# HamidGadirov/OpticalFlowSciVis

Hardware: AMD Instinct MI355X
Metric: volume-pairs/sec, Flow-3D unsupervised train step (fwd+loss+bwd+AdamW) (higher is better)
Workload: dtype f32

## Files before the change

opticalflowscivis_amd/csrc/convtr.hip:

```cpp
#include <cstdint>
#include <cstdlib>

#include "common.hpp"

namespace {

typedef float f32x16 __attribute__((ext_vector_type(16)));

struct TP {
  int B, Cin, Cout;
  int CoutT;
  int Di, Hi, Wi;
  int Dout, Hout, Wout;
  int Dq, Hq, Wq;
  int tz, ty, tx;
  long long tiles;
  const float* slope;
  float* Z;
  int nslope;
  const float* addend;
  const float* Ybase;
  long long wslice;
#ifdef FS_ABLATION
  int ab = 0;
// ... 589 lines not shown
  const int qz = qz0 + wz, qy = qy0 + wy;
  if (qz < p.Dq && qy < p.Hq) {
    const size_t yvol = (size_t)p.Dout * p.Hout * p.Wout;
#pragma unroll
    for (int n = 0; n < 2; ++n) {
      const int qx = qx0 + 16 * n + col;
#pragma unroll
      for (int r = 0; r < 4; ++r) {
        const int co = 4 * kq + r;
        const bool ok = co < p.Cout;
        const int cc = ok ? co : 0;
        const float bv = (bias && ok) ? bias[cc] : 0.f;
        float v[8];
#pragma unroll
        for (int c = 0; c < 8; ++c) v[c] = acc[n][c][r] + bv;
        store8_quad(Y + ((size_t)b * p.Cout + cc) * yvol, v, qz, qy, qx, ok, p,
                    p.Z ? p.Z + ((size_t)b * p.Cout + cc) * yvol : nullptr, p.Z ? p.slope[p.nslope == 1 ? 0 : cc] : 0.f);
      }
    }
  }
}

constexpr int p8_ws_ci(int rt) { return 128 * rt + 16; }
__host__ __device__ constexpr int p8_k(int par, int d) { return par == 0 ? (d == 0 ? 1 : 3) : (d == 0 ? 0 : 2); }

#ifdef FS_TR_STAMPS
__device__ unsigned long long fs_tr_dbg[4 * 8];
#define TSTAMP(i) do { const unsigned long long now_ = __builtin_amdgcn_s_memtime(); dt[i] += now_ - tprev; tprev = now_; } while (0)
#else
#define TSTAMP(i) do { } while (0)
#endif

template <int RT, int NT, int CINP>
__global__ __launch_bounds__(512, 2) void convtr_p8_kernel(const float* __restrict__ X, const float* __restrict__ Wt,
                                                        const float* __restrict__ bias, float* __restrict__ Y,
                                                        TP p, int per) {
  constexpr int CI = 4, XB = 16 * (NT - 1);
  constexpr int ZT = 3, YT = 3, XP = XB + 16;
  constexpr int PS = YT * XP;
  constexpr int CHS = ZT * PS + ((ZT * PS) % 32 == 16 ? 0 : 16);
  constexpr int NX = CI * CHS;
  constexpr int NXL = (NX + 255) / 256 * 256;
  constexpr int WSCI = p8_ws_ci(RT);
  constexpr int NW = CINP * WSCI;
  constexpr int NWL = (NW + 255) / 256 * 256;
  static_assert((NWL + 2 * NXL) * 4 <= 160 * 1024, "weights + two input buffers fit the CU's LDS");
  static_assert(NT % 2 == 1, "tiles are processed in pairs + one");
  __shared__ __attribute__((aligned(16))) float lds[NWL + 2 * NXL];

  const int t = threadIdx.x, lane = t & 63;
  const int wave = __builtin_amdgcn_readfirstlane(t >> 6);
  const int wv = wave & 3;
  const long long t0 = (long long)blockIdx.x * per, t1 = min(t0 + per, p.tiles);
  const size_t xvol = (size_t)p.Di * p.Hi * p.Wi;
  auto decode = [&](long long tile, int& b, int& qz0, int& qy0, int& q0) {
    const int txi = (int)(tile % p.tx); tile /= p.tx;
    const int tyi = (int)(tile % p.ty); tile /= p.ty;
    const int tzi = (int)(tile % p.tz);
    b = (int)(tile / p.tz);
    qz0 = tzi * 2; qy0 = tyi * 2; q0 = txi * XB;
  };

  if (wave >= 4) {
#if defined(__HIP_DEVICE_COMPILE__)
    __builtin_amdgcn_s_setprio(3);
    constexpr int NXW = (NXL / 256 + 3) / 4, NWW = (NWL / 256 + 3) / 4;
    {
      __amdgpu_buffer_rsrc_t rw = __builtin_amdgcn_make_buffer_rsrc((void*)Wt, (short)0, (p.Cin + 3) / 4 * 4 * WSCI * 4,
                                                                     0x00020000);
#pragma unroll
      for (int k = 0; k < NWW; ++k)
        if (256 * (wv + 4 * k) < NWL)
          __builtin_amdgcn_raw_ptr_buffer_load_lds(rw, (lds_ptr_t)(lds + 256 * (wv + 4 * k)), 16,
                                                   (unsigned)(256 * (wv + 4 * k) + 4 * lane) * 4u, 0, 0, 0);
    }
    unsigned xoff[NXW];
    int b = 0;
    auto offsets = [&](long long tile) {
      int qz0, qy0, q0;
      decode(tile, b, qz0, qy0, q0);
#pragma unroll
      for (int k = 0; k < NXW; ++k) {
        const int i = 256 * (wv + 4 * k) + 4 * lane;
        const int c = i / CHS, r1 = i - c * CHS;
        const int z = r1 / PS, r2 = r1 - z * PS;
        const int y = r2 / XP, x = r2 - y * XP;
        const int gz = qz0 - 1 + z, gy = qy0 - 1 + y, gx = q0 - 4 + x;
        const bool ok = i < NX && z < ZT && gz >= 0 && gz < p.Di && gy >= 0 && gy < p.Hi && gx >= 0 && gx < p.Wi;
// ... 38 lines not shown

  const int col = lane & 15, kq = lane >> 4;
  const int wz = wv >> 1, wy = wv & 1;
  const int bBo = NWL + kq * CHS + (wz + 1) * PS + (wy + 1) * XP + (col + 4);
  __builtin_amdgcn_s_barrier();
  int buf = 0;
#ifdef FS_TR_STAMPS
  unsigned long long dt[8] = {0, 0, 0, 0, 0, 0, 0, 0};
  unsigned long long tprev = __builtin_amdgcn_s_memtime();
#endif
  for (long long tile = t0; tile < t1; ++tile) {
    int b, qz0, qy0, q0;
    decode(tile, b, qz0, qy0, q0);
    const int qend = (q0 + XB >= p.Wi) ? p.Wi + 1 : q0 + XB;
    f32x4 acc[RT][NT];
#pragma unroll
    for (int rt = 0; rt < RT; ++rt)
#pragma unroll
      for (int n = 0; n < NT; ++n)
#pragma unroll
        for (int r = 0; r < 4; ++r) acc[rt][n][r] = 0.f;

    for (int c0 = 0; c0 < p.Cin; c0 += CI) {
      const float* aB = lds + (size_t)(c0 + kq) * WSCI + col;
      float av[8][RT];
#pragma unroll
      for (int d = 0; d < 8; ++d)
#pragma unroll
        for (int rt = 0; rt < RT; ++rt) av[d][rt] = aB[(d * RT + rt) * 16];
      const float* bB = lds + bBo + buf * NXL;
      float xa[2][8], xb[2][8];
      auto load_x = [&](int n, float (&xn)[8]) {
#pragma unroll
        for (int d = 0; d < 8; ++d) xn[d] = bB[16 * n - ((d >> 2) & 1) * PS - ((d >> 1) & 1) * XP - (d & 1)];
      };
      auto mma_pair = [&](int n, const float (&x0)[8], const float (&x1)[8], bool two) {
#pragma unroll
        for (int d = 0; d < 8; ++d)
#pragma unroll
          for (int rt = 0; rt < RT; ++rt) {
            acc[rt][n] = __builtin_amdgcn_mfma_f32_16x16x4f32(av[d][rt], x0[d], acc[rt][n], 0, 0, 0);
            if (two) acc[rt][n + 1] = __builtin_amdgcn_mfma_f32_16x16x4f32(av[d][rt], x1[d], acc[rt][n + 1], 0, 0, 0);
          }
      };
      load_x(0, xa[0]);
      if (NT > 1) load_x(1, xa[1]);
#pragma unroll
      for (int n = 0; n < NT; n += 4) {
        if (n + 2 < NT) { load_x(n + 2, xb[0]); if (n + 3 < NT) load_x(n + 3, xb[1]); }
        __builtin_amdgcn_sched_barrier(0);
        mma_pair(n, xa[0], xa[1], n + 1 < NT);
        if (n + 2 < NT) {
          if (n + 4 < NT) { load_x(n + 4, xa[0]); if (n + 5 < NT) load_x(n + 5, xa[1]); }
          __builtin_amdgcn_sched_barrier(0);
          mma_pair(n + 2, xb[0], xb[1], n + 3 < NT);
        }
      }
      TSTAMP(0);
      __builtin_amdgcn_s_barrier();
      TSTAMP(1);
      buf ^= 1;
    }

    const int qz = qz0 + wz, qy = qy0 + wy;
    if (qz <= p.Di && qy <= p.Hi) {
      const size_t yvol = (size_t)p.Dout * p.Hout * p.Wout;
      const bool evn = (col & 1) == 0;
      const int slot = 4 * (kq & 1) + (evn ? 0 : 1) + 2 * (lane >> 5);
#pragma unroll
      for (int rt = 0; rt < RT; ++rt) {
        const int item = 8 * rt + slot;
        const int pzy = item / p.Cout, co = item - pzy * p.Cout;
        const int zo = 2 * qz - (pzy >> 1), yo = 2 * qy - (pzy & 1);
        const bool iok = item < 4 * p.Cout && zo >= 0 && zo < p.Dout && yo >= 0 && yo < p.Hout;
        const float bv = (bias && iok) ? bias[co] : 0.f;
        float* __restrict__ row = Y + (((size_t)b * p.Cout + (iok ? co : 0)) * p.Dout + (iok ? zo : 0)) * ((size_t)p.Hout * p.Wout) +
                                  (size_t)(iok ? yo : 0) * p.Wout;
        const float* __restrict__ arow = p.addend ? p.addend + (row - Y) : nullptr;
// ... 147 lines not shown
}

template <int CO>
void launch_valu(const float* x, const float* w, const float* bias, float* y, const TP& p, hipStream_t st) {
  constexpr int NP = 2;
  const long long nq = (long long)p.B * p.Dq * ((p.Hq + NP - 1) / NP) * p.Wq;
  hipLaunchKernelGGL((convtr_valu_kernel<CO, NP>), dim3((unsigned)((nq + 255) / 256)), dim3(256), 0, st, x, w, bias,
                     y, p);
}

}

#ifdef FS_TR_STAMPS
extern "C" int fs_debug_tr_stamps(unsigned long long* out) {
  return hipMemcpyFromSymbol(out, HIP_SYMBOL(fs_tr_dbg), sizeof(unsigned long long) * 32) == hipSuccess ? 0 : 1;
}
#endif

extern "C" long long fs_conv3d_tr_ws_floats(int Cin, int Cout) {
  if (Cin < 1 || Cout < 1 || (Cout > 32 && (Cout % 32 != 0 || Cout > 128))) return -1;
  const int slices = Cout > 32 ? Cout / 32 : 1;
  if (Cout > 32) Cout = 32;
  const long long cinp = (Cin + 3) / 4 * 4;
  const long long p8 = Cout <= 12 ? cinp * p8_ws_ci(Cout <= 2 ? 1 : (Cout <= 6 ? 3 : 6)) : 0;
  long long cls = Cout <= 6 ? 0 : cinp * 64 * (Cout <= 16 ? 16 : 32);
  if (Cout > 16 && t3_slab_words(Cin) > cls) cls = t3_slab_words(Cin);
  if (Cout <= 16 && t3_slab_words16(Cin) > cls) cls = t3_slab_words16(Cin);
  return (p8 > cls ? p8 : cls) * slices;
}

static int conv3d_tr_slice(const float* x, const float* w, const float* bias, const float* slope, int nslope,
                          const float* addend, float* y, float* z, float* ws, int B, int Cin, int Cout, int Di,
                          int Hi, int Wi, int Dout, int Hout, int Wout, fs_stream_t stream, int CoutT = 0, int slices = 1,
                          WprepPlan* plan = nullptr) {
  FS_REQUIRE_PTR(x);
  if (plan == nullptr) FS_REQUIRE_PTR(y);
  if (z != nullptr && (slope == nullptr || (nslope != 1 && nslope != Cout))) return FS_ERR_ARG;
  if (B < 1 || Cin < 1 || Cout < 1 || Di < 1 || Hi < 1 || Wi < 1) return FS_ERR_SHAPE;
  if (Cout > 32) return FS_ERR_ARG;
  if (CoutT == 0) CoutT = Cout;
  if ((Dout != 2 * Di && Dout != 2 * Di + 1) || (Hout != 2 * Hi && Hout != 2 * Hi + 1) ||
      (Wout != 2 * Wi && Wout != 2 * Wi + 1))
    return FS_ERR_SHAPE;
  if ((long long)Di * Hi * Wi >= (1ll << 31) || (long long)Dout * Hout * Wout >= (1ll << 31))
    return FS_ERR_SHAPE;
  if ((long long)4 * Di * Hi * Wi * 4 >= (1ll << 32)) return FS_ERR_SHAPE;
  TP p;
  p.B = B; p.Cin = Cin; p.Cout = Cout; p.CoutT = CoutT; p.Di = Di; p.Hi = Hi; p.Wi = Wi;
  p.Dout = Dout; p.Hout = Hout; p.Wout = Wout;
  p.Dq = (Dout + 1) / 2; p.Hq = (Hout + 1) / 2; p.Wq = (Wout + 1) / 2;
  p.slope = slope; p.Z = z; p.nslope = nslope;
  p.addend = addend; p.Ybase = y;
  p.wslice = 0;
  hipStream_t st = (hipStream_t)stream;
  if ((long long)B * p.Dq * p.Hq * p.Wq >= (1ll << 31) * 256) return FS_ERR_SHAPE;
  static const bool reg_only = FS_AB_ENV("FLOWSCI_TR_REG");
  static const bool p8_all = FS_AB_ENV("FLOWSCI_TR_P8_ALL");
  static const bool s3_small = FS_AB_ENV("FLOWSCI_TR_S3_SMALL");
  if (!s3_small && Cout <= (p8_all ? 12 : 6) && !reg_only && z == nullptr && ws != nullptr && Cin <= (Cout <= 6 ? 64 : 32) && Dout == 2 * Di && Hout == 2 * Hi &&
      Wout == 2 * Wi && Wi % 4 == 0 && (((uintptr_t)x | (uintptr_t)ws) & 15) == 0 &&
      (long long)4 * Di * Hi * Wi * 4 < (1ll << 31)) {
    const int rt = Cout <= 2 ? 1 : (Cout <= 6 ? 3 : 6);
    const bool wide = Wi > 64 && rt < 6;
    p.tz = fs::cdiv(Di + 1, 2); p.ty = fs::cdiv(Hi + 1, 2); p.tx = fs::cdiv(Wi, wide ? 128 : 64);
    p.tiles = (long long)B * p.tz * p.ty * p.tx;
    if (p.tiles >= 16 && p.tiles < (1ll << 31)) {
      const int cinp = (Cin + 3) / 4 * 4;
      wprep_do(wprep_job(FS_WPREP_P8, w, ws, (long long)cinp * p8_ws_ci(rt), Cin, Cout, cinp, rt), plan, st);
      if (plan != nullptr) return FS_OK;
      if (Cin > 32) {
        if (rt == 1) { if (wide) launch_p8<1, 9, 64>(x, ws, bias, y, p, st); else launch_p8<1, 5, 64>(x, ws, bias, y, p, st); }
        else { if (wide) launch_p8<3, 9, 64>(x, ws, bias, y, p, st); else launch_p8<3, 5, 64>(x, ws, bias, y, p, st); }
      } else if (rt == 1) { if (wide) launch_p8<1, 9>(x, ws, bias, y, p, st); else launch_p8<1, 5>(x, ws, bias, y, p, st); }
      else if (rt == 3) { if (wide) launch_p8<3, 9>(x, ws, bias, y, p, st); else launch_p8<3, 5>(x, ws, bias, y, p, st); }
      else launch_p8<6, 5>(x, ws, bias, y, p, st);
      FS_LAUNCH_CHECK();
      return FS_OK;
    }
  }
  if (Cout <= 6 && !s3_small) {
    if (plan != nullptr) return FS_OK;
    if (w == nullptr) return FS_ERR_NULLPTR;
    if (Cout == 1) launch_valu<1>(x, w, bias, y, p, st);
    else if (Cout <= 2) launch_valu<2>(x, w, bias, y, p, st);
    else if (Cout <= 4) launch_valu<4>(x, w, bias, y, p, st);
    else launch_valu<6>(x, w, bias, y, p, st);
    FS_LAUNCH_CHECK();
    return FS_OK;
  }
  FS_REQUIRE_PTR(ws);
  const int cinp = (Cin + 3) / 4 * 4;
// ... 115 lines not shown
```

opticalflowscivis_amd/csrc/convtr_s3.hpp:

```cpp
#pragma once

typedef __bf16 t3_bf16x8 __attribute__((ext_vector_type(8)));
typedef unsigned t3_u32x4 __attribute__((ext_vector_type(4)));
typedef unsigned t3_u32x2 __attribute__((ext_vector_type(2)));
typedef int t3_i32x4 __attribute__((ext_vector_type(4)));
typedef const volatile __attribute__((address_space(3))) t3_u32x2* t3_lds_v64;

constexpr int T3_TZ = 2, T3_TY = 3, T3_TW = 32;
constexpr int T3_NMW = 8, T3_NLW = 4;
constexpr int T3_ZT = T3_TZ + 2, T3_YT = T3_TY + 2, T3_XP = 40;
constexpr int T3_NROW = T3_ZT * T3_YT;
constexpr int T3_NQ = T3_XP / 4;
constexpr int T3_ROWB = T3_XP * 8;
constexpr int T3_PIECEB = (T3_NROW + 1) * T3_ROWB;
constexpr int T3_INB = 3 * T3_PIECEB;
constexpr int T3_WB32 = 8 * 2 * 3 * 1024;
constexpr int T3_WORDS32 = T3_WB32 / 4;
static_assert(T3_NROW * T3_NQ <= 64 * T3_NLW, "one (row, piece) item per loader lane");

inline long long t3_slab_words(int Cin) { return (long long)((Cin + 3) / 4) * T3_WORDS32; }
constexpr int T3_WB16 = 8 * 3 * 1024;
inline long long t3_slab_words16(int Cin) { return (long long)((Cin + 3) / 4) * (T3_WB16 / 4); }

template <bool M16>
__global__ __launch_bounds__(64 * (T3_NMW + T3_NLW), 1) void convtr_s3_kernel(const float* __restrict__ X,
                                                                             const unsigned* __restrict__ Ws_,
                                                                             const float* __restrict__ bias_,
                                                                             float* __restrict__ Y_, TP p) {
  constexpr int NMW = T3_NMW, NLW = T3_NLW;
  constexpr int WOFF = 2 * T3_INB;
  constexpr int T3_WB = M16 ? T3_WB16 : T3_WB32;
  [[maybe_unused]] constexpr int T3_WORDS = T3_WB / 4;
  constexpr int NWW = T3_WB / 1024 / NLW;
  constexpr int STG1 = 4 * 256 * 16;
  constexpr int NSTG = M16 ? 2 : 1;
  constexpr int STGB = NSTG * STG1;
  static_assert(WOFF + 2 * T3_WB + STGB + 256 <= 160 * 1024, "the stages fit the CU's LDS");
  __shared__ __attribute__((aligned(16))) unsigned char lds[WOFF + 2 * T3_WB + STGB + 256];
  float* const sBias = reinterpret_cast<float*>(lds + WOFF + 2 * T3_WB + STGB);
  float* const sSlope = sBias + 32;

  const float* wd = reinterpret_cast<const float*>(Ws_);
  const float* bias = bias_;
  float* Y = Y_;
  tr_slice(p, wd, bias, Y);
// ... 59 lines not shown
        else
          asm volatile("s_nop 4\n\ts_mov_b32 m0, %0\n\ts_nop 0\n\tbuffer_load_dwordx4 %1, %2, 0 offen lds" ::"s"(m0v), "v"(goffA), "s"(r) : "memory");
      }
    };
    auto advance = [&]() {
      if (++l_s == NS) { l_s = 0; if (l_i + 1 < nbr) { ++l_i; l_brick(); } }
    };
    unsigned woff[NWW];
#pragma unroll
    for (int k = 0; k < NWW; ++k) {
      woff[k] = (unsigned)(1024 * (lw + NLW * k) + 16 * lane);
      asm volatile("" : "+v"(woff[k]));
    }
    auto issue_wdma = [&](int s, int buf) {
      const unsigned* src = Ws + (size_t)s * T3_WORDS;
      __amdgpu_buffer_rsrc_t rw = __builtin_amdgcn_make_buffer_rsrc((void*)src, (short)0, T3_WB, 0x00020000);
      unsigned char* dst = lds + WOFF + buf * T3_WB;
#pragma unroll
      for (int k = 0; k < NWW; ++k) {
        const int i = lw + NLW * k;
        __builtin_amdgcn_raw_ptr_buffer_load_lds(rw, (lds_ptr_t)(dst + 1024 * i), 16, woff[k], 0, 0, 0);
      }
    };
    auto convert = [&](int buf, const t3_u32x4 (&ld)[4]) {
      unsigned char* dst = lds + buf * T3_INB + loff;
      const unsigned u[4][4] = {{ld[0].x, ld[0].y, ld[0].z, ld[0].w}, {ld[1].x, ld[1].y, ld[1].z, ld[1].w},
                                {ld[2].x, ld[2].y, ld[2].z, ld[2].w}, {ld[3].x, ld[3].y, ld[3].z, ld[3].w}};
      unsigned h[3][4][2];
#pragma unroll
      for (int i = 0; i < 4; ++i)
#pragma unroll
        for (int cp = 0; cp < 2; ++cp) {
          float ra = __uint_as_float(u[2 * cp][i]), rc = __uint_as_float(u[2 * cp + 1][i]);
          h[0][i][cp] = s3_pack(ra, rc);
          ra -= __uint_as_float(h[0][i][cp] << 16); rc -= __uint_as_float(h[0][i][cp] & 0xffff0000u);
          asm volatile("" : "+v"(ra), "+v"(rc));
          h[1][i][cp] = s3_pack(ra, rc);
          ra -= __uint_as_float(h[1][i][cp] << 16); rc -= __uint_as_float(h[1][i][cp] & 0xffff0000u);
          asm volatile("" : "+v"(ra), "+v"(rc));
          h[2][i][cp] = s3_pack(ra, rc);
        }
#pragma unroll
      for (int pc = 0; pc < 3; ++pc) {
        const t3_u32x4 v0 = {h[pc][0][0], h[pc][0][1], h[pc][1][0], h[pc][1][1]};
        const t3_u32x4 v1 = {h[pc][2][0], h[pc][2][1], h[pc][3][0], h[pc][3][1]};
        *reinterpret_cast<t3_u32x4*>(dst + pc * T3_PIECEB) = v0;
        *reinterpret_cast<t3_u32x4*>(dst + pc * T3_PIECEB + 16) = v1;
      }
    };
    const int total = nbr * NS;
    issue_stage(0);
    if constexpr (NSTG == 2) {
      if (total > 1) { advance(); issue_stage(1); }
    }
    int s = 0;
    for (int g = 0; g < total; ++g) {
      if (NSTG == 2 && g + 1 < total) asm volatile("s_waitcnt vmcnt(4)" ::: "memory");
      else asm volatile("s_waitcnt vmcnt(0)" ::: "memory");
      t3_u32x4 ld[4];
      const unsigned char* sp = stg + (NSTG == 2 ? (g & 1) * STG1 : 0);
#pragma unroll
      for (int c = 0; c < 4; ++c) ld[c] = *reinterpret_cast<const t3_u32x4*>(sp + c * 4096);
      asm volatile("s_waitcnt lgkmcnt(0)" ::: "memory");
      __builtin_amdgcn_sched_barrier(0);
      issue_wdma(s, g & 1);
      const bool more = g + NSTG < total;
      if (more) {
        advance();
        issue_stage(NSTG == 2 ? (g & 1) : 0);
      }
      __builtin_amdgcn_sched_barrier(0);
#ifdef FS_ABLATION
// ... 38 lines not shown
        __builtin_amdgcn_s_barrier();
        const unsigned char* sb = lds + (gs & 1) * T3_INB + bO;
        const unsigned char* sw = lds + (gs & 1) * T3_WB + aO;
#ifdef FS_ABLATION
        if (p.ab & 64) continue;
#endif
        auto read_b = [&](int px, int i, t3_bf16x8 (&bq)[3]) {
          const int y = i >> 1, h = i & 1;
#pragma unroll
          for (int pc = 0; pc < 3; ++pc) {
            const unsigned char* q = sb + pc * T3_PIECEB + y * T3_ROWB + (16 * h + px) * 8;
            const t3_u32x2 lo = *(t3_lds_v64)(lds_ptr_t)(q + dz0), hi = *(t3_lds_v64)(lds_ptr_t)(q + dz1);
            const t3_u32x4 v = {lo.x, lo.y, hi.x, hi.y};
            bq[pc] = __builtin_bit_cast(t3_bf16x8, v);
          }
        };
#pragma unroll
        for (int px = 0; px < 2; ++px) {
          t3_bf16x8 a[3], b0[3], b1[3];
#pragma unroll
          for (int pc = 0; pc < 3; ++pc)
            a[pc] = __builtin_bit_cast(t3_bf16x8, *reinterpret_cast<const t3_u32x4*>(sw + (px * 3 + pc) * 1024));
          read_b(px, 0, b0);
          constexpr int PA[6] = {2, 0, 1, 1, 0, 0}, PB[6] = {0, 2, 1, 0, 1, 0};
#pragma unroll
          for (int i = 0; i < 2 * T3_TY; i += 2) {
            read_b(px, i + 1, b1);
            __builtin_amdgcn_sched_barrier(0);
#ifdef FS_ABLATION
            if (!(p.ab & 128))
#endif
#pragma unroll
            for (int q6 = 0; q6 < 6; ++q6)
              acc[px][i >> 1][i & 1] = __builtin_amdgcn_mfma_f32_16x16x32_bf16(a[PA[q6]], b0[PB[q6]], acc[px][i >> 1][i & 1], 0, 0, 0);
            if (i + 2 < 2 * T3_TY) read_b(px, i + 2, b0);
            __builtin_amdgcn_sched_barrier(0);
#ifdef FS_ABLATION
            if (!(p.ab & 128))
#endif
#pragma unroll
            for (int q6 = 0; q6 < 6; ++q6)
              acc[px][(i + 1) >> 1][(i + 1) & 1] = __builtin_amdgcn_mfma_f32_16x16x32_bf16(a[PA[q6]], b1[PB[q6]], acc[px][(i + 1) >> 1][(i + 1) & 1], 0, 0, 0);
          }
        }
      }
#ifdef FS_ABLATION
      if (p.ab & 4) continue;
#endif
      int b, qz0, qy0, qx0;
      brick_origin(bi, b, qz0, qy0, qx0);
      const int qz = qz0 + g;
      if (qz >= p.Dq) continue;
      const unsigned yv = (unsigned)yvol;
      const size_t sb0 = (size_t)b * p.CoutT * yvol;
      float* const yb = Y + sb0;
      const float* const ab = p.addend != nullptr ? p.addend + (Y - p.Ybase) + sb0 : nullptr;
      float* const zb = p.Z != nullptr ? p.Z + sb0 : nullptr;
      int kqe = kq;
      asm volatile("" : "+v"(kqe));
      const bool evn = (n16 & 1) == 0;
#pragma unroll
      for (int y = 0; y < T3_TY; ++y) {
        const int qy = qy0 + y;
        if (qy >= p.Hq) break;
#pragma unroll
// ... 64 lines not shown
        for (int px = 0; px < 2; ++px)
#pragma unroll
          for (int pc = 0; pc < 3; ++pc)
            a[px][pc] = __builtin_bit_cast(t3_bf16x8, *reinterpret_cast<const t3_u32x4*>(sw + ((px * 2 + az) * 3 + pc) * 1024));
#pragma unroll
        for (int y = 0; y < T3_TY; ++y) {
          t3_u32x2 P[3][3];
#pragma unroll
          for (int pc = 0; pc < 3; ++pc)
#pragma unroll
            for (int d = 0; d < 3; ++d)
              P[pc][d] = *(t3_lds_v64)(lds_ptr_t)(sb + dzr + pc * T3_PIECEB + y * T3_ROWB + (d - 1) * 8);
          t3_bf16x8 bq[2][3];
#pragma unroll
          for (int px = 0; px < 2; ++px)
#pragma unroll
            for (int pc = 0; pc < 3; ++pc) {
              const t3_u32x4 v = {P[pc][px].x, P[pc][px].y, P[pc][px + 1].x, P[pc][px + 1].y};
              bq[px][pc] = __builtin_bit_cast(t3_bf16x8, v);
            }
#ifdef FS_ABLATION
          if (p.ab & 128) continue;
#endif
          constexpr int PA[6] = {2, 0, 1, 1, 0, 0}, PB[6] = {0, 2, 1, 0, 1, 0};
#pragma unroll
          for (int q = 0; q < 6; ++q)
#pragma unroll
            for (int px = 0; px < 2; ++px)
              acc[px][y] = __builtin_amdgcn_mfma_f32_32x32x16_bf16(a[px][PA[q]], bq[px][PB[q]], acc[px][y], 0, 0, 0);
        }
      }
    }

#ifdef FS_ABLATION
    if (p.ab & 4) continue;
#endif
    int b, qz0, qy0, qx0;
    brick_origin(bi, b, qz0, qy0, qx0);
    const int qz = qz0 + g, qx = qx0 + col;
    if (qz >= p.Dq) continue;
    const unsigned yv = (unsigned)yvol;
    const size_t sb0 = (size_t)b * p.CoutT * yvol;
    float* const yb = Y + sb0;
    const float* const ab = p.addend != nullptr ? p.addend + (Y - p.Ybase) + sb0 : nullptr;
    float* const zb = p.Z != nullptr ? p.Z + sb0 : nullptr;
    int khe = kh;
    asm volatile("" : "+v"(khe));
    const unsigned khv = 4u * (unsigned)khe * yv;
    const bool evn = (col & 1) == 0;
    const int qxe = evn ? qx : qx - 1;
    const bool xin = qxe < p.Wq;
#pragma unroll
// ... 34 lines not shown
```

opticalflowscivis_amd/csrc/wprep.hpp:

```cpp
#pragma once

enum { FS_WPREP_FWD = 0, FS_WPREP_TR32 = 1, FS_WPREP_TR16 = 2, FS_WPREP_P8 = 3, FS_WPREP_WINO = 4, FS_WPREP_WINO4 = 5,
       FS_WPREP_WINO2D = 6, FS_WPREP_S3K4 = 7, FS_WPREP_TRS3 = 8, FS_WPREP_TRS3_16 = 9 };

__device__ __forceinline__ unsigned s3_pack(float a, float b) {
  typedef __bf16 bf16x2_t __attribute__((ext_vector_type(2)));
  const bf16x2_t h = {(__bf16)a, (__bf16)b};
  return __builtin_bit_cast(unsigned, h);
}

__device__ __forceinline__ unsigned wprep_s3_word(const FsWprepJob& j, int e) {
  const int Cout = j.p[0], Cin = j.p[1], CinP2 = j.p[2], CP = j.p[3];
  const float* __restrict__ w = j.w;
  const int kx = e & 3;
  int r = e >> 2;
  const int col = r % CP; r /= CP;
  const int kh = r & 1, kyp = (r >> 1) & 1; r >>= 2;
  const int piece = r % 3; r /= 3;
  const int kz = r & 3; r >>= 2;
  const int cp = r % CinP2, mg = r / CinP2;
  const int co = mg * CP + col, tap = (kz * 4 + 2 * kyp + kh) * 4 + kx;
  float v[2];
#pragma unroll
  for (int i = 0; i < 2; ++i) {
    const int ci = 2 * cp + i;
    float a = (co < Cout && ci < Cin) ? w[((size_t)co * Cin + ci) * 64 + tap] : 0.f;
    for (int q = 0; q < piece; ++q) a = a - (float)(__bf16)a;
    v[i] = a;
// ... 15 lines not shown
#pragma unroll
  for (int i = 0; i < 2; ++i) {
    const int ci = 4 * st + 2 * c2 + i;
    float a = (co < Cout && ci < Cin) ? w[((size_t)ci * CoutT + co) * 64 + tap] : 0.f;
    for (int q = 0; q < piece; ++q) a = a - (float)(__bf16)a;
    v[i] = a;
  }
  return s3_pack(v[0], v[1]);
}
__device__ __forceinline__ unsigned wprep_t3_word16(const FsWprepJob& j, int e) {
  const int Cin = j.p[0], Cout = j.p[1], CoutT = j.p[3];
  const float* __restrict__ w = j.w;
  const int c2 = e & 1, az = (e >> 1) & 1, co = (e >> 2) & 15, kq = (e >> 6) & 3;
  int r = e >> 8;
  const int piece = r % 3; r /= 3;
  const int cls = r & 7, st = r >> 3;
  const int pz = cls >> 2, py = (cls >> 1) & 1, px = cls & 1;
  const int tap = (wprep_p8_k(pz, az) * 4 + wprep_p8_k(py, kq >> 1)) * 4 + wprep_p8_k(px, kq & 1);
  float v[2];
#pragma unroll
  for (int i = 0; i < 2; ++i) {
    const int ci = 4 * st + 2 * c2 + i;
    float a = (co < Cout && ci < Cin) ? w[((size_t)ci * CoutT + co) * 64 + tap] : 0.f;
    for (int q = 0; q < piece; ++q) a = a - (float)(__bf16)a;
    v[i] = a;
  }
  return s3_pack(v[0], v[1]);
}
constexpr int FS_WINO_UCH = 9 * 4 * 64 + 16;
constexpr int FS_WINO4_UCH = 9 * 6 * 64;
constexpr int FS_WINO2D_UCH = 3 * 24 * 64;

__device__ __forceinline__ float wprep_g43(const float (&g)[3], int tt) {
  switch (tt) {
    case 0: return 0.25f * g[0];
    case 1: return (-1.f / 6.f) * ((g[0] + g[2]) + g[1]);
    case 2: return (-1.f / 6.f) * ((g[0] + g[2]) - g[1]);
    case 3: return (1.f / 24.f) * g[0] + ((1.f / 12.f) * g[1] + (1.f / 6.f) * g[2]);
    case 4: return (1.f / 24.f) * g[0] + ((-1.f / 12.f) * g[1] + (1.f / 6.f) * g[2]);
    default: return g[2];
  }
}

__device__ __forceinline__ float wprep_elem(const FsWprepJob& j, int e) {
  const float* __restrict__ w = j.w;
  switch (j.kind) {
// ... 43 lines not shown
    case FS_WPREP_WINO2D: {
      const int Cout = j.p[0], Cin = j.p[1], mode = j.p[3];
      const int ci = e / FS_WINO2D_UCH, i = e - ci * FS_WINO2D_UCH;
      if (ci >= Cin) return 0.f;
      const int kz = i / 1536, r = i - kz * 1536;
      const int ty = r / 384, r2 = r - ty * 384;
      const int tx = r2 >> 6, co = r2 & 63;
      if (co >= Cout) return 0.f;
      float u[3];
#pragma unroll
      for (int ky = 0; ky < 3; ++ky) {
        float g[3];
#pragma unroll
        for (int kx = 0; kx < 3; ++kx) {
          const int tap = (kz * 3 + ky) * 3 + kx;
          g[kx] = mode ? w[((size_t)ci * Cout + co) * 27 + (26 - tap)] : w[((size_t)co * Cin + ci) * 27 + tap];
        }
        u[ky] = wprep_g43(g, tx);
      }
      return ty == 0 ? u[0] : ty == 1 ? 0.5f * ((u[0] + u[1]) + u[2]) : ty == 2 ? 0.5f * ((u[0] - u[1]) + u[2]) : u[2];
    }
    default: {
      const int Cin = j.p[0], Cout = j.p[1], RT = j.p[3];
      const int wsci = 128 * RT + 16;
      const int ci = e / wsci, i = e - ci * wsci;
      if (i >= 128 * RT || ci >= Cin) return 0.f;
      const int d = i / (16 * RT), r2 = i - d * 16 * RT;
      const int rt = r2 >> 4, row = r2 & 15;
      const int px = row >> 3, item = 8 * rt + (row & 7);
      if (item >= 4 * Cout) return 0.f;
      const int pzy = item / Cout, co = item - pzy * Cout;
      const int kz = wprep_p8_k(pzy >> 1, (d >> 2) & 1), ky = wprep_p8_k(pzy & 1, (d >> 1) & 1), kx = wprep_p8_k(px, d & 1);
      return w[((size_t)ci * Cout + co) * 64 + (kz * 4 + ky) * 4 + kx];
    }
  }
}

__device__ __forceinline__ void wprep_wino2d_blocks(const FsWprepJob& j, int first, int stride) {
  __shared__ float g9[64 * 9 + 64];
  const int Cout = j.p[0], Cin = j.p[1], CinP = j.p[2], mode = j.p[3];
  const float* __restrict__ w = j.w;
  const int t = threadIdx.x;
  for (int blk = first; blk < CinP * 3; blk += stride) {
    const int ci = blk / 3, kz = blk - ci * 3;
    __syncthreads();
    for (int i = t; i < 64 * 9; i += 256) {
// ... 72 lines not shown
```

Baseline: 31.64.

## Use split-bf16x3 MFMA path for small-Cin, small-Cout parity-8 transposed conv

```diff
diff --git a/opticalflowscivis_amd/csrc/convtr.hip b/opticalflowscivis_amd/csrc/convtr.hip
--- a/opticalflowscivis_amd/csrc/convtr.hip
+++ b/opticalflowscivis_amd/csrc/convtr.hip
@@ -635,6 +635,7 @@
 }
 
 constexpr int p8_ws_ci(int rt) { return 128 * rt + 16; }
+constexpr long long p8_split_words(int cinp, int rt) { return (long long)(cinp / 4) * rt * 768; }
 __host__ __device__ constexpr int p8_k(int par, int d) { return par == 0 ? (d == 0 ? 1 : 3) : (d == 0 ? 0 : 2); }
 
 #ifdef FS_TR_STAMPS
@@ -657,9 +658,27 @@
   constexpr int WSCI = p8_ws_ci(RT);
   constexpr int NW = CINP * WSCI;
   constexpr int NWL = (NW + 255) / 256 * 256;
-  static_assert((NWL + 2 * NXL) * 4 <= 160 * 1024, "weights + two input buffers fit the CU's LDS");
   static_assert(NT % 2 == 1, "tiles are processed in pairs + one");
-  __shared__ __attribute__((aligned(16))) float lds[NWL + 2 * NXL];
+  constexpr bool S3 = CINP == 32 && RT <= 3;
+  constexpr int S_ROWB = XP * 8;
+  constexpr int S_PIECEB = ZT * YT * S_ROWB + 64;
+  constexpr int S_IMGB = 3 * S_PIECEB;
+  constexpr int S_WTB = (CINP / CI) * RT * 3 * 1024;
+  constexpr int S_NQ = XP / 4;
+  constexpr int S_NITEM = ZT * YT * S_NQ;
+  [[maybe_unused]] constexpr int S_NSLOT = (S_NITEM + 255) / 256;
+  constexpr int S_STGB = (S_NITEM + 63) / 64 * 4096;
+  constexpr int S_BYTES = S_WTB + 2 * S_IMGB + S_STGB;
+#ifdef FS_ABLATION
+  constexpr int LDSF = (S3 && S_BYTES / 4 > NWL + 2 * NXL) ? S_BYTES / 4 : NWL + 2 * NXL;
+  const bool s3 = S3 && !(p.ab & 256);
+#else
+  constexpr int LDSF = S3 ? S_BYTES / 4 : NWL + 2 * NXL;
+  constexpr bool s3 = S3;
+#endif
+  static_assert(LDSF * 4 <= 160 * 1024, "weights + the input stages fit the CU's LDS");
+  __shared__ __attribute__((aligned(16))) float lds[LDSF];
+  [[maybe_unused]] unsigned char* const ldsb = reinterpret_cast<unsigned char*>(lds);
 
   const int t = threadIdx.x, lane = t & 63;
   const int wave = __builtin_amdgcn_readfirstlane(t >> 6);
@@ -677,6 +696,91 @@
   if (wave >= 4) {
 #if defined(__HIP_DEVICE_COMPILE__)
     __builtin_amdgcn_s_setprio(3);
+    if constexpr (S3) {
+      if (s3) {
+        {
+          __amdgpu_buffer_rsrc_t rw = __builtin_amdgcn_make_buffer_rsrc((void*)Wt, (short)0, (p.Cin + 3) / 4 * RT * 3072, 0x00020000);
+#pragma unroll
+          for (int k = 0; k < S_WTB / 4096; ++k)
+            __builtin_amdgcn_raw_ptr_buffer_load_lds(rw, (lds_ptr_t)(ldsb + 1024 * (wv + 4 * k)), 16,
+                                                     (unsigned)(1024 * (wv + 4 * k) + 16 * lane), 0, 0, 0);
+        }
+        unsigned char* const stg = ldsb + S_WTB + 2 * S_IMGB;
+        const unsigned volB = (unsigned)(xvol * 4u);
+        unsigned xoff[S_NSLOT];
+        int b = 0;
+        auto offsets = [&](long long tile) {
+          int qz0, qy0, q0;
+          decode(tile, b, qz0, qy0, q0);
+#pragma unroll
+          for (int sl = 0; sl < S_NSLOT; ++sl) {
+            const int item = 256 * sl + 64 * wv + lane;
+            const int row = item / S_NQ, jq = item - row * S_NQ;
+            const int z = row / YT, y = row - z * YT;
+            const int gz = qz0 - 1 + z, gy = qy0 - 1 + y, gx = q0 - 4 + 4 * jq;
+            const bool ok = item < S_NITEM && gz >= 0 && gz < p.Di && gy >= 0 && gy < p.Hi && gx >= 0 && gx + 3 < p.Wi;
+            xoff[sl] = ok ? (((unsigned)gz * p.Hi + gy) * p.Wi + gx) * 4u : DMA_OOB;
+          }
+        };
+        auto stage = [&](int c0) {
+#pragma unroll
+          for (int c = 0; c < CI; ++c) {
+            const bool in = c0 + c < p.Cin;
+            __amdgpu_buffer_rsrc_t rx = __builtin_amdgcn_make_buffer_rsrc(
+                (void*)(X + ((size_t)b * p.Cin + (in ? c0 + c : 0)) * xvol), (short)0, in ? (int)volB : 0, 0x00020000);
+#pragma unroll
+            for (int sl = 0; sl < S_NSLOT; ++sl)
+              if (256 * sl + 64 * wv < S_NITEM)
+                __builtin_amdgcn_raw_ptr_buffer_load_lds(rx, (lds_ptr_t)(stg + (4 * sl + wv) * 4096 + c * 1024), 16, xoff[sl], 0, 0, 0);
+          }
+        };
+        long long rtile = t0;
+        int rc0 = 0;
+        auto request_next = [&]() {
+          if (rc0 + CI < p.Cin) rc0 += CI;
+          else if (rtile + 1 < t1) { ++rtile; rc0 = 0; offsets(rtile); }
+          else return;
+          stage(rc0);
+        };
+        auto take = [&](int buf) {
+          asm volatile("s_waitcnt vmcnt(0)" ::: "memory");
+          t3_u32x4 ld[S_NSLOT][4];
+#pragma unroll
+          for (int sl = 0; sl < S_NSLOT; ++sl)
+            if (256 * sl + 64 * wv < S_NITEM)
+#pragma unroll
+              for (int c = 0; c < CI; ++c)
+                ld[sl][c] = *reinterpret_cast<const t3_u32x4*>(stg + (4 * sl + wv) * 4096 + c * 1024 + 16 * lane);
+          asm volatile("s_waitcnt lgkmcnt(0)" ::: "memory");
+          __builtin_amdgcn_sched_barrier(0);
+          request_next();
+          __builtin_amdgcn_sched_barrier(0);
+#pragma unroll
+          for (int sl = 0; sl < S_NSLOT; ++sl)
+            if (256 * sl + 64 * wv < S_NITEM) {
+              const int item = 256 * sl + 64 * wv + lane;
+              const int row = item / S_NQ, jq = item - row * S_NQ;
+              if (item < S_NITEM) t3_split_store(ld[sl], ldsb + S_WTB + buf * S_IMGB + row * S_ROWB + jq * 32, S_PIECEB);
+            }
+          asm volatile("s_waitcnt lgkmcnt(0)" ::: "memory");
+        };
+        if (t0 < t1) {
+          offsets(t0);
+          stage(0);
+          take(0);
+        }
+        asm volatile("s_waitcnt vmcnt(0)" ::: "memory");
+        __builtin_amdgcn_s_barrier();
+        int buf = 0;
+        for (long long tile = t0; tile < t1; ++tile)
+          for (int c0 = 0; c0 < p.Cin; c0 += CI) {
+            if (c0 + CI < p.Cin || tile + 1 < t1) take(buf ^ 1);
+            __builtin_amdgcn_s_barrier();
+            buf ^= 1;
+          }
+        return;
+      }
+    }
     constexpr int NXW = (NXL / 256 + 3) / 4, NWW = (NWL / 256 + 3) / 4;
     {
       __amdgpu_buffer_rsrc_t rw = __builtin_amdgcn_make_buffer_rsrc((void*)Wt, (short)0, (p.Cin + 3) / 4 * 4 * WSCI * 4,
@@ -761,38 +865,98 @@
         for (int r = 0; r < 4; ++r) acc[rt][n][r] = 0.f;
 
     for (int c0 = 0; c0 < p.Cin; c0 += CI) {
-      const float* aB = lds + (size_t)(c0 + kq) * WSCI + col;
-      float av[8][RT];
-#pragma unroll
-      for (int d = 0; d < 8; ++d)
-#pragma unroll
-        for (int rt = 0; rt < RT; ++rt) av[d][rt] = aB[(d * RT + rt) * 16];
-      const float* bB = lds + bBo + buf * NXL;
-      float xa[2][8], xb[2][8];
-      auto load_x = [&](int n, float (&xn)[8]) {
-#pragma unroll
-        for (int d = 0; d < 8; ++d) xn[d] = bB[16 * n - ((d >> 2) & 1) * PS - ((d >> 1) & 1) * XP - (d & 1)];
-      };
-      auto mma_pair = [&](int n, const float (&x0)[8], const float (&x1)[8], bool two) {
+      bool done = false;
+      if constexpr (S3) {
+        if (s3) {
+          const unsigned char* wt = ldsb + (c0 / CI) * RT * 3072 + 16 * lane;
+          t3_bf16x8 a[RT][3];
+#pragma unroll
+          for (int rt = 0; rt < RT; ++rt)
+#pragma unroll
+            for (int pc = 0; pc < 3; ++pc)
+              a[rt][pc] = __builtin_bit_cast(t3_bf16x8, *reinterpret_cast<const t3_u32x4*>(wt + (rt * 3 + pc) * 1024));
+          const unsigned char* img = ldsb + S_WTB + buf * S_IMGB +
+                                     (((wz + 1 - (kq >> 1)) * YT + (wy + 1 - (kq & 1))) * XP + col + 3) * 8;
+          auto load_b = [&](int n, t3_bf16x8 (&bq)[3]) {
+#pragma unroll
+            for (int pc = 0; pc < 3; ++pc) {
+              const unsigned char* q = img + pc * S_PIECEB + n * 128;
+              const t3_u32x2 lo = *(t3_lds_v64)(lds_ptr_t)q, hi = *(t3_lds_v64)(lds_ptr_t)(q + 8);
+              const t3_u32x4 v = {lo.x, lo.y, hi.x, hi.y};
+              bq[pc] = __builtin_bit_cast(t3_bf16x8, v);
+            }
+          };
+          auto mma_pair = [&](int n, const t3_bf16x8 (&b0)[3], const t3_bf16x8 (&b1)[3], bool two) {
+#pragma unroll
+            for (int q6 = 0; q6 < 6; ++q6)
+#pragma unroll
+              for (int rt = 0; rt < RT; ++rt) {
+                acc[rt][n] = __builtin_amdgcn_mfma_f32_16x16x32_bf16(a[rt][T3_PA[q6]], b0[T3_PB[q6]], acc[rt][n], 0, 0, 0);
+                if (two) acc[rt][n + 1] = __builtin_amdgcn_mfma_f32_16x16x32_bf16(a[rt][T3_PA[q6]], b1[T3_PB[q6]], acc[rt][n + 1], 0, 0, 0);
+              }
+          };
+          t3_bf16x8 ba[2][3], bb[2][3];
+          load_b(0, ba[0]);
+          if (NT > 1) load_b(1, ba[1]);
+#pragma unroll
+          for (int n = 0; n < NT; n += 4) {
+            if (n + 2 < NT) { load_b(n + 2, bb[0]); if (n + 3 < NT) load_b(n + 3, bb[1]); }
+            __builtin_amdgcn_sched_barrier(0);
+            mma_pair(n, ba[0], ba[1], n + 1 < NT);
+            if (n + 2 < NT) {
+              if (n + 4 < NT) { load_b(n + 4, ba[0]); if (n + 5 < NT) load_b(n + 5, ba[1]); }
+              __builtin_amdgcn_sched_barrier(0);
+              mma_pair(n + 2, bb[0], bb[1], n + 3 < NT);
+            }
+          }
+          done = true;
+        }
+      }
+      if (!done) {
+        const float* aB = lds + (size_t)(c0 + kq) * WSCI + col;
+        float av[8][RT];
 #pragma unroll
         for (int d = 0; d < 8; ++d)
 #pragma unroll
-          for (int rt = 0; rt < RT; ++rt) {
-            acc[rt][n] = __builtin_amdgcn_mfma_f32_16x16x4f32(av[d][rt], x0[d], acc[rt][n], 0, 0, 0);
-            if (two) acc[rt][n + 1] = __builtin_amdgcn_mfma_f32_16x16x4f32(av[d][rt], x1[d], acc[rt][n + 1], 0, 0, 0);
+          for (int rt = 0; rt < RT; ++rt) av[d][rt] = aB[(d * RT + rt) * 16];
+        const float* bB = lds + bBo + buf * NXL;
+        float xa[2][8], xb[2][8];
+        auto load_x = [&](int n, float (&xn)[8]) {
+#pragma unroll
+          for (int d = 0; d < 8; ++d) xn[d] = bB[16 * n - ((d >> 2) & 1) * PS - ((d >> 1) & 1) * XP - (d & 1)];
+        };
+        auto mma_pair = [&](int n, const float (&x0)[8], const float (&x1)[8], bool two) {
+#pragma unroll
+          for (int d = 0; d < 8; ++d)
+#pragma unroll
+            for (int rt = 0; rt < RT; ++rt) {
+              acc[rt][n] = __builtin_amdgcn_mfma_f32_16x16x4f32(av[d][rt], x0[d], acc[rt][n], 0, 0, 0);
+              if (two) acc[rt][n + 1] = __builtin_amdgcn_mfma_f32_16x16x4f32(av[d][rt], x1[d], acc[rt][n + 1], 0, 0, 0);
+            }
+        };
+        if constexpr (RT == 6) {
+#pragma unroll
+          for (int n = 0; n < NT; n += 2) {
+            load_x(n, xa[0]);
+            if (n + 1 < NT) load_x(n + 1, xa[1]);
+            __builtin_amdgcn_sched_barrier(0);
+            mma_pair(n, xa[0], xa[1], n + 1 < NT);
+            __builtin_amdgcn_sched_barrier(0);
           }
-      };
-      load_x(0, xa[0]);
-      if (NT > 1) load_x(1, xa[1]);
-#pragma unroll
-      for (int n = 0; n < NT; n += 4) {
-        if (n + 2 < NT) { load_x(n + 2, xb[0]); if (n + 3 < NT) load_x(n + 3, xb[1]); }
-        __builtin_amdgcn_sched_barrier(0);
-        mma_pair(n, xa[0], xa[1], n + 1 < NT);
-        if (n + 2 < NT) {
-          if (n + 4 < NT) { load_x(n + 4, xa[0]); if (n + 5 < NT) load_x(n + 5, xa[1]); }
-          __builtin_amdgcn_sched_barrier(0);
-          mma_pair(n + 2, xb[0], xb[1], n + 3 < NT);
+        } else {
+          load_x(0, xa[0]);
+          if (NT > 1) load_x(1, xa[1]);
+#pragma unroll
+          for (int n = 0; n < NT; n += 4) {
+            if (n + 2 < NT) { load_x(n + 2, xb[0]); if (n + 3 < NT) load_x(n + 3, xb[1]); }
+            __builtin_amdgcn_sched_barrier(0);
+            mma_pair(n, xa[0], xa[1], n + 1 < NT);
+            if (n + 2 < NT) {
+              if (n + 4 < NT) { load_x(n + 4, xa[0]); if (n + 5 < NT) load_x(n + 5, xa[1]); }
+              __builtin_amdgcn_sched_barrier(0);
+              mma_pair(n + 2, xb[0], xb[1], n + 3 < NT);
+            }
+          }
         }
       }
       TSTAMP(0);
@@ -986,7 +1150,8 @@
   const int slices = Cout > 32 ? Cout / 32 : 1;
   if (Cout > 32) Cout = 32;
   const long long cinp = (Cin + 3) / 4 * 4;
-  const long long p8 = Cout <= 12 ? cinp * p8_ws_ci(Cout <= 2 ? 1 : (Cout <= 6 ? 3 : 6)) : 0;
+  long long p8 = Cout <= 12 ? cinp * p8_ws_ci(Cout <= 2 ? 1 : (Cout <= 6 ? 3 : 6)) : 0;
+  if (Cout <= 6 && cinp <= 32 && p8_split_words((int)cinp, Cout <= 2 ? 1 : 3) > p8) p8 = p8_split_words((int)cinp, Cout <= 2 ? 1 : 3);
   long long cls = Cout <= 6 ? 0 : cinp * 64 * (Cout <= 16 ? 16 : 32);
   if (Cout > 16 && t3_slab_words(Cin) > cls) cls = t3_slab_words(Cin);
   if (Cout <= 16 && t3_slab_words16(Cin) > cls) cls = t3_slab_words16(Cin);
@@ -1030,7 +1195,13 @@
     p.tiles = (long long)B * p.tz * p.ty * p.tx;
     if (p.tiles >= 16 && p.tiles < (1ll << 31)) {
       const int cinp = (Cin + 3) / 4 * 4;
-      wprep_do(wprep_job(FS_WPREP_P8, w, ws, (long long)cinp * p8_ws_ci(rt), Cin, Cout, cinp, rt), plan, st);
+      static const bool p8_no_s3 = FS_AB_ENV("FLOWSCI_TR_P8_NO_S3");
+      const bool split = Cin <= 32 && rt <= 3 && !p8_no_s3;
+#ifdef FS_ABLATION
+      if (!split) p.ab = 256;
+#endif
+      wprep_do(wprep_job(FS_WPREP_P8, w, ws, split ? p8_split_words(cinp, rt) : (long long)cinp * p8_ws_ci(rt), Cin, Cout, cinp, rt,
+                         split ? 1 : 0), plan, st);
       if (plan != nullptr) return FS_OK;
       if (Cin > 32) {
         if (rt == 1) { if (wide) launch_p8<1, 9, 64>(x, ws, bias, y, p, st); else launch_p8<1, 5, 64>(x, ws, bias, y, p, st); }
diff --git a/opticalflowscivis_amd/csrc/convtr_s3.hpp b/opticalflowscivis_amd/csrc/convtr_s3.hpp
--- a/opticalflowscivis_amd/csrc/convtr_s3.hpp
+++ b/opticalflowscivis_amd/csrc/convtr_s3.hpp
@@ -21,6 +21,34 @@
 inline long long t3_slab_words(int Cin) { return (long long)((Cin + 3) / 4) * T3_WORDS32; }
 constexpr int T3_WB16 = 8 * 3 * 1024;
 inline long long t3_slab_words16(int Cin) { return (long long)((Cin + 3) / 4) * (T3_WB16 / 4); }
+
+constexpr int T3_PA[6] = {2, 0, 1, 1, 0, 0}, T3_PB[6] = {0, 2, 1, 0, 1, 0};
+
+__device__ __forceinline__ void t3_split_store(const t3_u32x4 (&ld)[4], unsigned char* dst, int pieceb) {
+  const unsigned u[4][4] = {{ld[0].x, ld[0].y, ld[0].z, ld[0].w}, {ld[1].x, ld[1].y, ld[1].z, ld[1].w},
+                            {ld[2].x, ld[2].y, ld[2].z, ld[2].w}, {ld[3].x, ld[3].y, ld[3].z, ld[3].w}};
+  unsigned h[3][4][2];
+#pragma unroll
+  for (int i = 0; i < 4; ++i)
+#pragma unroll
+    for (int cp = 0; cp < 2; ++cp) {
+      float ra = __uint_as_float(u[2 * cp][i]), rc = __uint_as_float(u[2 * cp + 1][i]);
+      h[0][i][cp] = s3_pack(ra, rc);
+      ra -= __uint_as_float(h[0][i][cp] << 16); rc -= __uint_as_float(h[0][i][cp] & 0xffff0000u);
+      asm volatile("" : "+v"(ra), "+v"(rc));
+      h[1][i][cp] = s3_pack(ra, rc);
+      ra -= __uint_as_float(h[1][i][cp] << 16); rc -= __uint_as_float(h[1][i][cp] & 0xffff0000u);
+      asm volatile("" : "+v"(ra), "+v"(rc));
+      h[2][i][cp] = s3_pack(ra, rc);
+    }
+#pragma unroll
+  for (int pc = 0; pc < 3; ++pc) {
+    const t3_u32x4 v0 = {h[pc][0][0], h[pc][0][1], h[pc][1][0], h[pc][1][1]};
+    const t3_u32x4 v1 = {h[pc][2][0], h[pc][2][1], h[pc][3][0], h[pc][3][1]};
+    *reinterpret_cast<t3_u32x4*>(dst + pc * pieceb) = v0;
+    *reinterpret_cast<t3_u32x4*>(dst + pc * pieceb + 16) = v1;
+  }
+}
 
 template <bool M16>
 __global__ __launch_bounds__(64 * (T3_NMW + T3_NLW), 1) void convtr_s3_kernel(const float* __restrict__ X,
@@ -126,32 +154,7 @@
         __builtin_amdgcn_raw_ptr_buffer_load_lds(rw, (lds_ptr_t)(dst + 1024 * i), 16, woff[k], 0, 0, 0);
       }
     };
-    auto convert = [&](int buf, const t3_u32x4 (&ld)[4]) {
-      unsigned char* dst = lds + buf * T3_INB + loff;
-      const unsigned u[4][4] = {{ld[0].x, ld[0].y, ld[0].z, ld[0].w}, {ld[1].x, ld[1].y, ld[1].z, ld[1].w},
-                                {ld[2].x, ld[2].y, ld[2].z, ld[2].w}, {ld[3].x, ld[3].y, ld[3].z, ld[3].w}};
-      unsigned h[3][4][2];
-#pragma unroll
-      for (int i = 0; i < 4; ++i)
-#pragma unroll
-        for (int cp = 0; cp < 2; ++cp) {
-          float ra = __uint_as_float(u[2 * cp][i]), rc = __uint_as_float(u[2 * cp + 1][i]);
-          h[0][i][cp] = s3_pack(ra, rc);
-          ra -= __uint_as_float(h[0][i][cp] << 16); rc -= __uint_as_float(h[0][i][cp] & 0xffff0000u);
-          asm volatile("" : "+v"(ra), "+v"(rc));
-          h[1][i][cp] = s3_pack(ra, rc);
-          ra -= __uint_as_float(h[1][i][cp] << 16); rc -= __uint_as_float(h[1][i][cp] & 0xffff0000u);
-          asm volatile("" : "+v"(ra), "+v"(rc));
-          h[2][i][cp] = s3_pack(ra, rc);
-        }
-#pragma unroll
-      for (int pc = 0; pc < 3; ++pc) {
-        const t3_u32x4 v0 = {h[pc][0][0], h[pc][0][1], h[pc][1][0], h[pc][1][1]};
-        const t3_u32x4 v1 = {h[pc][2][0], h[pc][2][1], h[pc][3][0], h[pc][3][1]};
-        *reinterpret_cast<t3_u32x4*>(dst + pc * T3_PIECEB) = v0;
-        *reinterpret_cast<t3_u32x4*>(dst + pc * T3_PIECEB + 16) = v1;
-      }
-    };
+    auto convert = [&](int buf, const t3_u32x4 (&ld)[4]) { t3_split_store(ld, lds + buf * T3_INB + loff, T3_PIECEB); };
     const int total = nbr * NS;
     issue_stage(0);
     if constexpr (NSTG == 2) {
@@ -236,7 +239,6 @@
           for (int pc = 0; pc < 3; ++pc)
             a[pc] = __builtin_bit_cast(t3_bf16x8, *reinterpret_cast<const t3_u32x4*>(sw + (px * 3 + pc) * 1024));
           read_b(px, 0, b0);
-          constexpr int PA[6] = {2, 0, 1, 1, 0, 0}, PB[6] = {0, 2, 1, 0, 1, 0};
 #pragma unroll
           for (int i = 0; i < 2 * T3_TY; i += 2) {
             read_b(px, i + 1, b1);
@@ -246,7 +248,7 @@
 #endif
 #pragma unroll
             for (int q6 = 0; q6 < 6; ++q6)
-              acc[px][i >> 1][i & 1] = __builtin_amdgcn_mfma_f32_16x16x32_bf16(a[PA[q6]], b0[PB[q6]], acc[px][i >> 1][i & 1], 0, 0, 0);
+              acc[px][i >> 1][i & 1] = __builtin_amdgcn_mfma_f32_16x16x32_bf16(a[T3_PA[q6]], b0[T3_PB[q6]], acc[px][i >> 1][i & 1], 0, 0, 0);
             if (i + 2 < 2 * T3_TY) read_b(px, i + 2, b0);
             __builtin_amdgcn_sched_barrier(0);
 #ifdef FS_ABLATION
@@ -254,7 +256,7 @@
 #endif
 #pragma unroll
             for (int q6 = 0; q6 < 6; ++q6)
-              acc[px][(i + 1) >> 1][(i + 1) & 1] = __builtin_amdgcn_mfma_f32_16x16x32_bf16(a[PA[q6]], b1[PB[q6]], acc[px][(i + 1) >> 1][(i + 1) & 1], 0, 0, 0);
+              acc[px][(i + 1) >> 1][(i + 1) & 1] = __builtin_amdgcn_mfma_f32_16x16x32_bf16(a[T3_PA[q6]], b1[T3_PB[q6]], acc[px][(i + 1) >> 1][(i + 1) & 1], 0, 0, 0);
           }
         }
       }
@@ -365,12 +367,11 @@
 #ifdef FS_ABLATION
           if (p.ab & 128) continue;
 #endif
-          constexpr int PA[6] = {2, 0, 1, 1, 0, 0}, PB[6] = {0, 2, 1, 0, 1, 0};
 #pragma unroll
           for (int q = 0; q < 6; ++q)
 #pragma unroll
             for (int px = 0; px < 2; ++px)
-              acc[px][y] = __builtin_amdgcn_mfma_f32_32x32x16_bf16(a[px][PA[q]], bq[px][PB[q]], acc[px][y], 0, 0, 0);
+              acc[px][y] = __builtin_amdgcn_mfma_f32_32x32x16_bf16(a[px][T3_PA[q]], bq[px][T3_PB[q]], acc[px][y], 0, 0, 0);
         }
       }
     }
diff --git a/opticalflowscivis_amd/csrc/wprep.hpp b/opticalflowscivis_amd/csrc/wprep.hpp
--- a/opticalflowscivis_amd/csrc/wprep.hpp
+++ b/opticalflowscivis_amd/csrc/wprep.hpp
@@ -3,7 +3,7 @@
 enum { FS_WPREP_FWD = 0, FS_WPREP_TR32 = 1, FS_WPREP_TR16 = 2, FS_WPREP_P8 = 3, FS_WPREP_WINO = 4, FS_WPREP_WINO4 = 5,
        FS_WPREP_WINO2D = 6, FS_WPREP_S3K4 = 7, FS_WPREP_TRS3 = 8, FS_WPREP_TRS3_16 = 9 };
 
-__device__ __forceinline__ unsigned s3_pack(float a, float b) {
+__host__ __device__ __forceinline__ unsigned s3_pack(float a, float b) {
   typedef __bf16 bf16x2_t __attribute__((ext_vector_type(2)));
   const bf16x2_t h = {(__bf16)a, (__bf16)b};
   return __builtin_bit_cast(unsigned, h);
@@ -65,6 +65,27 @@
   for (int i = 0; i < 2; ++i) {
     const int ci = 4 * st + 2 * c2 + i;
     float a = (co < Cout && ci < Cin) ? w[((size_t)ci * CoutT + co) * 64 + tap] : 0.f;
+    for (int q = 0; q < piece; ++q) a = a - (float)(__bf16)a;
+    v[i] = a;
+  }
+  return s3_pack(v[0], v[1]);
+}
+__host__ __device__ __forceinline__ unsigned wprep_p8s_word(const FsWprepJob& j, int e) {
+  const int Cin = j.p[0], Cout = j.p[1], RT = j.p[3];
+  const float* __restrict__ w = j.w;
+  const int cp = e & 1, xs = (e >> 1) & 1, row = (e >> 2) & 15, kq = (e >> 6) & 3;
+  int r = e >> 8;
+  const int piece = r % 3; r /= 3;
+  const int rt = r % RT, chunk = r / RT;
+  const int px = row >> 3, item = 8 * rt + (row & 7);
+  const bool iok = item < 4 * Cout;
+  const int pzy = iok ? item / Cout : 0, co = iok ? item - pzy * Cout : 0;
+  const int kz = wprep_p8_k(pzy >> 1, kq >> 1), ky = wprep_p8_k(pzy & 1, kq & 1), kx = wprep_p8_k(px, 1 - xs);
+  float v[2];
+#pragma unroll
+  for (int i = 0; i < 2; ++i) {
+    const int ci = 4 * chunk + 2 * cp + i;
+    float a = (iok && ci < Cin) ? w[((size_t)ci * Cout + co) * 64 + (kz * 4 + ky) * 4 + kx] : 0.f;
     for (int q = 0; q < piece; ++q) a = a - (float)(__bf16)a;
     v[i] = a;
   }
@@ -154,6 +175,7 @@
     }
     default: {
       const int Cin = j.p[0], Cout = j.p[1], RT = j.p[3];
+      if (j.p[4] != 0) return __builtin_bit_cast(float, wprep_p8s_word(j, e));
       const int wsci = 128 * RT + 16;
       const int ci = e / wsci, i = e - ci * wsci;
       if (i >= 128 * RT || ci >= Cin) return 0.f;
```

Result: faster. 32.22, median of 6 (+1.8%).
